# NVlabs/FB-BEV

Hardware: AMD Instinct MI355X
Metric: multi-cam samples/sec (forward view transformation: lift + voxel ranking + bev_pool_v2) (higher is better)
Workload: dtype f32

## Files before the change

fb_bev_amd/csrc/capi.hip:

```cpp
#include <stdio.h>
#include <stdlib.h>
#include <mutex>
#include "rt.h"
#include "pool_kernels.h"
#include "pool_bwd_kernels.h"
#include "rank_kernels.h"
#include "sort_kernels.h"
#include "msda_kernels.h"
#include "geom_kernels.h"
#include "da_kernels.h"
#include "history_kernels.h"
#include "norm_kernels.h"
#include "history_conv_kernels.h"
#include "history_fused_kernels.h"
#include "history_conv_x3_kernels.h"
#include "history_fused_x3_kernels.h"
#include "rows_linear_kernels.h"
#include "rows_linear_f32_kernels.h"
#include "da_fused_kernels.h"
#include "da_bwd_planes_kernels.h"
#include "msda_bwd_kernels.h"
#include "conv3d_kernels.h"
#include "det_kernels.h"
#include "occ_kernels.h"
// ... 102 lines not shown
}

extern "C" int fbbev_tokens_from_nchw_levels(const float* const* in, const int32_t* hw, int n_levels, float* out, int n_images, int C,
                                             const float* bias, int bias_rows, fbbev_stream_t stream_) {
    if (n_levels <= 0 || n_levels > 8 || n_images < 0 || C <= 0 || !in || !hw) return FBBEV_E_BADARG;
    if (bias && bias_rows <= 0) return FBBEV_E_BADARG;
    if (n_images == 0) return 0;
    if (!out) return FBBEV_E_BADARG;
    fbbev_token_levels lv;
    const int tc = (C + 31) / 32;
    long long start = 0, blocks = 0;
    for (int l = 0; l < 8; ++l) { lv.in[l] = nullptr; lv.out_off[l] = 0; lv.hw[l] = 1; lv.blk0[l] = 0; }
    for (int l = 0; l < n_levels; ++l) {
        if (hw[l] <= 0 || !in[l]) return FBBEV_E_BADARG;
        lv.in[l] = in[l]; lv.hw[l] = hw[l]; lv.out_off[l] = start * C; lv.blk0[l] = (int)blocks;
        start += hw[l];
        blocks += (long long)n_images * tc * ((hw[l] + 31) / 32);
        if (blocks >= (1ll << 31)) return FBBEV_E_UNSUPPORTED;
    }
    lv.blk0[n_levels] = (int)blocks;
    lv.n = n_levels;
    FBBEV_LAUNCH(k_nchw_to_nhwc_levels, blocks, 256, 0, (fbbev_rt_stream)stream_, lv, out, C, tc, start * C, bias, bias ? bias_rows : 1);
    FBBEV_CHECK_LAUNCH();
    return 0;
}

extern "C" int fbbev_tokens_from_nchw_pos(const float* in, float* out, int n_images, int C, int HW, long long out_image_stride,
                                          long long out_offset, const float* pos_bias, fbbev_stream_t stream_) {
    if (!pos_bias) return FBBEV_E_BADARG;
    return tokens_from_nchw_impl(in, out, n_images, C, HW, out_image_stride, out_offset, nullptr, 0, pos_bias, stream_);
}

extern "C" int fbbev_point_sampling(const float* xs, const float* ys, const float* zs, const float* rots,
                                    const float* trans, const float* intrins, const float* post_rots,
                                    const float* post_trans, const float* bda, int B, int N, int Y, int X,
                                    int Za, float ogfH, float ogfW, float* ref_cam, uint8_t* mask,
                                    float* qdepth, fbbev_stream_t stream_) {
    if (B <= 0 || N <= 0 || Y <= 0 || X <= 0 || Za <= 0 || !(ogfH > 0.f) || !(ogfW > 0.f)) return FBBEV_E_BADARG;
    if (!xs || !ys || !zs || !rots || !trans || !intrins || !post_rots || !post_trans || !bda || !ref_cam ||
        !mask || !qdepth) return FBBEV_E_BADARG;
    const long long npts = (long long)Y * X * Za;
    int ppt = 8;
    while (ppt > 1 && (npts + 256 * ppt - 1) / (256 * ppt) * B * N < 1024) ppt >>= 1;
    const long long chunks = (npts + 256 * ppt - 1) / (256 * ppt);
    if (chunks * B * N >= (1ll << 31) || ((uintptr_t)ref_cam & 7) != 0) return FBBEV_E_UNSUPPORTED;
    FBBEV_LAUNCH(k_point_sampling, chunks * B * N, 256, 0, (fbbev_rt_stream)stream_, xs, ys, zs, rots, trans,
                 intrins, post_rots, post_trans, bda, B, N, Y, X, Za, ogfH, ogfW, (int)chunks, ref_cam, mask,
                 qdepth, ppt);
    FBBEV_CHECK_LAUNCH();
    return 0;
}

static inline int key_bits(long long total_voxels) {
    int bits = 1;
    while ((1ll << bits) < total_voxels) ++bits;
    return bits;
}

static const int kSortTile[7] = {2048, 4096, 8192, 12288, 16384, 4096, 8192};
static int sort_variant_for(long long items) {
    for (int v = 0; v < 5; ++v)
        if ((items + kSortTile[v] - 1) / kSortTile[v] <= 256) return v;
    return 6;
}
static const int kIvTile[3] = {1024, 4096, 8192};
static int iv_variant_for(long long items) {
    for (int v = 0; v < 3; ++v)
        if ((items + kIvTile[v] - 1) / kIvTile[v] <= 256) return v;
    return 2;
}

static fbbev_fastdiv make_fastdiv(unsigned int d) {
    fbbev_fastdiv f;
    f.d = d; f.m = 0; f.sh = 0;
    if (d <= 1) { f.d = 1; return f; }
    unsigned int l = 0;
    while ((1ull << l) < d) ++l;
    f.m = (unsigned int)((((1ull << l) - d) << 32) / d + 1);
    f.sh = l - 1;
    return f;
}

struct rank_ws_layout {
    size_t keys_a, keys_t, vals_t, matrix, ctot, chunk_info, total;
    int v0, wgs0;
    int v1, wgs1;
    int vi, wgsi;
};

static rank_ws_layout rank_layout(long long n) {
    rank_ws_layout L;
    L.v0 = sort_variant_for(n);
    L.v1 = sort_variant_for((n + 1) / 2);
    L.vi = iv_variant_for((n + 1) / 2);
    if (const char* env = fbbev_env_str("FBBEV_RANK_SHAPE")) {
        int a = -1, b = -1, c = -1;
        if (sscanf(env, "%d,%d,%d", &a, &b, &c) == 3 && a >= 0 && a < 7 && b >= 0 && b < 7 && c >= 0 && c < 3) {
            L.v0 = a; L.v1 = b; L.vi = c;
        }
    }
    L.wgs0 = (int)((n + kSortTile[L.v0] - 1) / kSortTile[L.v0]);
    L.wgs1 = (int)((n + kSortTile[L.v1] - 1) / kSortTile[L.v1]);
    L.wgsi = (int)((n + kIvTile[L.vi] - 1) / kIvTile[L.vi]);
    size_t off = 0;
    L.keys_a = off; off = align_up(off + (size_t)n * 4, 256);
    L.keys_t = off; off = align_up(off + (size_t)n * 4, 256);
    L.vals_t = off; off = align_up(off + (size_t)n * 4, 256);
    const int rows = L.wgs0 > L.wgs1 ? L.wgs0 : L.wgs1;
    const size_t seg_rows = (size_t)(n / FBBEV_SEG_TILE) + 256 + 1;
    size_t mbytes = (size_t)rows * FBBEV_SORT_MAX_NB * 4;
    if (seg_rows * FBBEV_SEG_NB * 4 > mbytes) mbytes = seg_rows * FBBEV_SEG_NB * 4;
    L.matrix = off; off = align_up(off + mbytes, 256);
    L.ctot = off; off = align_up(off + seg_rows * 4, 256);
    L.chunk_info = off; off = align_up(off + (size_t)L.wgsi * 8, 256);
    L.total = off;
    return L;
}

#define FBBEV_SORT_DISPATCH(KERNEL, v, by_waves, grid, stream, ...)                                             \
    do {                                                                                                        \
        switch (v) {                                                                                            \
            case 0: FBBEV_LAUNCH((KERNEL<(by_waves) ? 4 : 256, 8>), grid, 256, 0, stream, __VA_ARGS__); break;   \
            case 1: FBBEV_LAUNCH((KERNEL<(by_waves) ? 16 : 1024, 4>), grid, 1024, 0, stream, __VA_ARGS__); break; \
            case 2: FBBEV_LAUNCH((KERNEL<(by_waves) ? 16 : 1024, 8>), grid, 1024, 0, stream, __VA_ARGS__); break; \
            case 3: FBBEV_LAUNCH((KERNEL<(by_waves) ? 16 : 1024, 12>), grid, 1024, 0, stream, __VA_ARGS__); break; \
            case 5: FBBEV_LAUNCH((KERNEL<(by_waves) ? 8 : 512, 8>), grid, 512, 0, stream, __VA_ARGS__); break;     \
            case 6: FBBEV_LAUNCH((KERNEL<(by_waves) ? 8 : 512, 16>), grid, 512, 0, stream, __VA_ARGS__); break;    \
            default: FBBEV_LAUNCH((KERNEL<(by_waves) ? 16 : 1024, 16>), grid, 1024, 0, stream, __VA_ARGS__); break; \
        }                                                                                                       \
    } while (0)

extern "C" size_t fbbev_rank_workspace_bytes(int64_t n_points) {
    if (n_points <= 0) return 256;
    return rank_layout(n_points).total;
}

static int rank_seg_mode() { FBBEV_KNOB_ONCE(int, m, fbbev_env_int("FBBEV_RANK_SEG", -1)); return m; }

static int rank_build_impl(const float* coor, const fbbev_cam_ptrs* cams, const float* frustum, int B, int N, int D,
                           int H, int W,
                           const float* lower3, const float* interval3, const float* grid_size3,
                           int32_t* ranks_bev, int32_t* ranks_depth, int32_t* ranks_feat,
                           int32_t* interval_starts, int32_t* interval_lengths, int32_t* interval_rank,
                           int32_t* counts, void* workspace, size_t workspace_bytes, fbbev_rt_stream stream,
                           const float* point_depth = nullptr, float depth_thr = 0.f, const int* skip = nullptr) {
    if (B <= 0 || N <= 0 || D <= 0 || H <= 0 || W <= 0) return FBBEV_E_BADARG;
    if (point_depth && cams) return FBBEV_E_UNSUPPORTED;
    if ((!coor && !cams) || !lower3 || !interval3 || !grid_size3 || !ranks_bev || !ranks_depth || !ranks_feat ||
        !interval_starts || !interval_lengths || !counts || !workspace) return FBBEV_E_BADARG;
    const long long n = (long long)B * N * D * H * W;
    if (n >= (1ll << 30)) return FBBEV_E_UNSUPPORTED;
    const rank_ws_layout L = rank_layout(n);
    if (workspace_bytes < L.total) return FBBEV_E_WORKSPACE;
    unsigned char* ws = static_cast<unsigned char*>(workspace);
    unsigned int* keys_a = reinterpret_cast<unsigned int*>(ws + L.keys_a);
    unsigned int* keys_t = reinterpret_cast<unsigned int*>(ws + L.keys_t);
    unsigned int* vals_t = reinterpret_cast<unsigned int*>(ws + L.vals_t);
    int* matrix = reinterpret_cast<int*>(ws + L.matrix);
    int2* chunk_info = reinterpret_cast<int2*>(ws + L.chunk_info);

    fbbev_grid_params gp;
    gp.lx = lower3[0]; gp.ly = lower3[1]; gp.lz = lower3[2];
    gp.ix = interval3[0]; gp.iy = interval3[1]; gp.iz = interval3[2];
    gp.gx = grid_size3[0]; gp.gy = grid_size3[1]; gp.gz = grid_size3[2];
    volatile float zy = gp.gz * gp.gy;
    volatile float zyx = zy * gp.gx;
    volatile float yx = gp.gy * gp.gx;
    gp.f_zyx = zyx; gp.f_yx = yx;
    const long long total_voxels = (long long)B * (long long)gp.gz * (long long)gp.gy * (long long)gp.gx;
    if (total_voxels <= 0 || total_voxels >= (1ll << 30)) return FBBEV_E_UNSUPPORTED;
    const int bits = key_bits(total_voxels + 128);
    struct { int passes, rb; } plan;
    plan.passes = (bits + FBBEV_SORT_MAX_RB - 1) / FBBEV_SORT_MAX_RB;
    plan.rb = (bits + plan.passes - 1) / plan.passes;
    if (plan.rb < 4) plan.rb = 4;
    const int rb = plan.rb;
    const int seg_mode = rank_seg_mode();
    const long long vps = total_voxels / B;
    const long long npb = n / B;
    const int lbits = key_bits(vps);
    const bool seg_legal = B <= 256 && total_voxels <= (1ll << 24) && lbits <= 2 * FBBEV_SEG_RB;
    const long long seg_cps = (npb + FBBEV_SEG_TILE - 1) / FBBEV_SEG_TILE;
    const bool seg = seg_legal && seg_mode != 0 &&
                     (seg_mode == 2 || ((lbits + FBBEV_SEG_RB - 1) / FBBEV_SEG_RB < plan.passes && seg_cps <= 64 && B * seg_cps >= 96));
    if (seg) {
        fbbev_seg sg;
        sg.npb = (int)npb; sg.cps = (int)((npb + FBBEV_SEG_TILE - 1) / FBBEV_SEG_TILE); sg.vps = (unsigned int)vps; sg.nseg = B;
        const int passes = (lbits + FBBEV_SEG_RB - 1) / FBBEV_SEG_RB;
        const int srb = (lbits + passes - 1) / passes < 4 ? 4 : (lbits + passes - 1) / passes;
        const int wgs = B * sg.cps;
        int* ctot = reinterpret_cast<int*>(ws + L.ctot);
        fbbev_geom_src gs;
        if (cams) { gs.cam = *cams; gs.frustum = frustum; gs.gp = gp; }
        else { gs.cam = fbbev_cam_ptrs(); gs.frustum = nullptr; gs.gp = gp; }
        if (cams) FBBEV_LAUNCH((k_keys_hist_seg<true>), wgs, FBBEV_SEG_NT, 0, stream, gs, (const float*)nullptr, gp, (const float*)nullptr, 0.f,
                               sg, srb, skip, keys_a, matrix, ctot);
        else FBBEV_LAUNCH((k_keys_hist_seg<false>), wgs, FBBEV_SEG_NT, 0, stream, gs, coor, gp, point_depth, depth_thr, sg, srb, skip, keys_a,
                          matrix, ctot);
        FBBEV_CHECK_LAUNCH();
        const unsigned int* kin = keys_a;
        const unsigned int* vin = nullptr;
        static const int pairs = fbbev_env_int("FBBEV_RANK_PAIRS", 1);
        for (int p = 0; p < passes; ++p) {
            const bool to_out = p == passes - 1;
            const int pm = pairs ? ((p > 0 ? 1 : 0) | (to_out ? 0 : 2)) : 0;
            unsigned int* ko = to_out ? reinterpret_cast<unsigned int*>(ranks_bev) : keys_t;
            unsigned int* vo = to_out ? reinterpret_cast<unsigned int*>(ranks_depth) : vals_t;
            if (p > 0) {
                FBBEV_LAUNCH(k_sort_hist_seg, wgs, FBBEV_SEG_NT, 0, stream, kin, (const int*)ctot, sg, p * srb, srb, skip, matrix,
                             (pm & 1) ? 2 : 1);
                FBBEV_CHECK_LAUNCH();
            }
            static const int swz = fbbev_env_int("FBBEV_RANK_XCD_SWIZZLE", 1);
            const int sw = (swz && B >= 8) ? 1 : 0;
            FBBEV_LAUNCH(k_sort_scatter_seg, sw ? (wgs + 7) / 8 * 8 : wgs, FBBEV_SEG_NT, 0, stream, kin, vin, (const int*)matrix,
                         (const int*)ctot, sg, p, srb, skip, ko, vo, counts, sw, pm);
            FBBEV_CHECK_LAUNCH();
            kin = ko; vin = vo;
        }
    } else {
    if (cams) {
            fbbev_geom_src gs;
            gs.cam = *cams; gs.frustum = frustum; gs.gp = gp;
            FBBEV_SORT_DISPATCH(k_keys_hist_geom, L.v0, false, L.wgs0, stream, gs, n, rb, skip, keys_a, matrix);
        } else {
            FBBEV_SORT_DISPATCH(k_keys_hist_coor, L.v0, false, L.wgs0, stream, coor, n, n / B, gp, point_depth, depth_thr, rb, keys_a, matrix);
        }
        FBBEV_CHECK_LAUNCH();
        const unsigned int* kin = keys_a;
        const unsigned int* vin = nullptr;
        for (int p = 0; p < plan.passes; ++p) {
            const bool to_out = ((plan.passes - 1 - p) % 2) == 0;
            unsigned int* ko = to_out ? reinterpret_cast<unsigned int*>(ranks_bev) : keys_t;
            unsigned int* vo = to_out ? reinterpret_cast<unsigned int*>(ranks_depth) : vals_t;
            const int v = p == 0 ? L.v0 : L.v1, wgs = p == 0 ? L.wgs0 : L.wgs1;
            if (p > 0) {
                FBBEV_SORT_DISPATCH(k_sort_hist, v, false, wgs, stream, kin, (const int*)counts, p * rb, rb, skip, matrix);
                FBBEV_CHECK_LAUNCH();
            }
            static const int swz = fbbev_env_int("FBBEV_RANK_XCD_SWIZZLE", 1);
            const bool sw = swz == 2 && p == 0;
            FBBEV_SORT_DISPATCH(k_sort_scatter, v, true, sw ? (wgs + 7) / 8 * 8 : wgs, stream, kin, vin, n, (const int*)matrix, p, rb, skip,
                                ko, vo, counts, sw ? wgs : 0);
            FBBEV_CHECK_LAUNCH();
            kin = ko; vin = vo;
        }
}
    const unsigned int* keys = reinterpret_cast<const unsigned int*>(ranks_bev);
    const unsigned int* vals = reinterpret_cast<const unsigned int*>(ranks_depth);
    const fbbev_fastdiv div_dhw = make_fastdiv((unsigned int)((long long)D * H * W)), div_hw = make_fastdiv((unsigned int)(H * W));
    switch (L.vi) {
        case 0:
            FBBEV_LAUNCH((k_interval_count<4, 4>), L.wgsi, 256, 0, stream, keys, (const int*)counts, skip, chunk_info);
            FBBEV_LAUNCH((k_interval_write<4, 4>), L.wgsi, 256, (size_t)2 * 4 * 256 * 4, stream, keys, vals, div_dhw, div_hw, (const int2*)chunk_info, skip,
                         ranks_feat, interval_starts, interval_lengths, interval_rank, counts);
            break;
        case 1:
            FBBEV_LAUNCH((k_interval_count<16, 4>), L.wgsi, 1024, 0, stream, keys, (const int*)counts, skip, chunk_info);
            FBBEV_LAUNCH((k_interval_write<16, 4>), L.wgsi, 1024, (size_t)2 * 4 * 1024 * 4, stream, keys, vals, div_dhw, div_hw, (const int2*)chunk_info, skip,
                         ranks_feat, interval_starts, interval_lengths, interval_rank, counts);
            break;
        default:
            FBBEV_LAUNCH((k_interval_count<16, 8>), L.wgsi, 1024, 0, stream, keys, (const int*)counts, skip, chunk_info);
            FBBEV_LAUNCH((k_interval_write<16, 8>), L.wgsi, 1024, (size_t)2 * 8 * 1024 * 4, stream, keys, vals, div_dhw, div_hw, (const int2*)chunk_info, skip,
                         ranks_feat, interval_starts, interval_lengths, interval_rank, counts);
            break;
    }
    FBBEV_CHECK_LAUNCH();
    return 0;
}

extern "C" int fbbev_rank_build(const float* coor, int B, int N, int D, int H, int W,
                                const float* lower3, const float* interval3,
                                const float* grid_size3, int32_t* ranks_bev, int32_t* ranks_depth,
                                int32_t* ranks_feat, int32_t* interval_starts,
                                int32_t* interval_lengths, int32_t* interval_rank, int32_t* counts,
                                void* workspace, size_t workspace_bytes, fbbev_stream_t stream_) {
    if (!coor) return FBBEV_E_BADARG;
    return rank_build_impl(coor, nullptr, nullptr, B, N, D, H, W, lower3, interval3, grid_size3, ranks_bev, ranks_depth,
                           ranks_feat, interval_starts, interval_lengths, interval_rank, counts, workspace,
                           workspace_bytes, (fbbev_rt_stream)stream_);
}

extern "C" int fbbev_rank_build_depth(const float* coor, const float* depth, float depth_threshold, int B, int N, int D,
                                      int H, int W, const float* lower3, const float* interval3,
                                      const float* grid_size3, int32_t* ranks_bev, int32_t* ranks_depth,
                                      int32_t* ranks_feat, int32_t* interval_starts, int32_t* interval_lengths,
                                      int32_t* interval_rank, int32_t* counts, void* workspace, size_t workspace_bytes,
                                      fbbev_stream_t stream_) {
    if (!coor || !depth) return FBBEV_E_BADARG;
    return rank_build_impl(coor, nullptr, nullptr, B, N, D, H, W, lower3, interval3, grid_size3, ranks_bev, ranks_depth,
                           ranks_feat, interval_starts, interval_lengths, interval_rank, counts, workspace,
                           workspace_bytes, (fbbev_rt_stream)stream_, depth, depth_threshold);
}

static int lift_rank_build_impl(const float* frustum, const float* xs, const float* ys, const float* ds,
                                const float* rots, const float* trans, const float* intrins, const float* post_rots,
                                const float* post_trans, const float* bda, int B, int N, int D, int H, int W,
                                const float* lower3, const float* interval3, const float* grid_size3,
// ... 3383 lines not shown
```

fb_bev_amd/csrc/rank_kernels.h:

```cpp
#pragma once
#include "rt.h"


struct fbbev_grid_params {
    float lx, ly, lz;
    float ix, iy, iz;
    float gx, gy, gz;
    float f_yx, f_zyx;
};

__device__ __forceinline__ unsigned int fbbev_rank_key(float cx, float cy, float cz, const fbbev_grid_params& gp,
                                                       float bf, unsigned int sentinel) {
    const float fx = __fdiv_rn(fbbev_sub(cx, gp.lx), gp.ix);
    const float fy = __fdiv_rn(fbbev_sub(cy, gp.ly), gp.iy);
    const float fz = __fdiv_rn(fbbev_sub(cz, gp.lz), gp.iz);
    const bool finite = (fx == fx) && (fy == fy) && (fz == fz) && fabsf(fx) < 2.0e9f &&
                        fabsf(fy) < 2.0e9f && fabsf(fz) < 2.0e9f;
    const int vx = finite ? (int)fx : -1;
    const int vy = finite ? (int)fy : -1;
    const int vz = finite ? (int)fz : -1;
    const bool kept = finite && vx >= 0 && vy >= 0 && vz >= 0 && (float)vx < gp.gx &&
                      (float)vy < gp.gy && (float)vz < gp.gz;
    float r = fbbev_mul(bf, gp.f_zyx);
    r = fbbev_add(r, fbbev_mul((float)vz, gp.f_yx));
// ... 115 lines not shown
                 int* __restrict__ interval_starts, int* __restrict__ interval_lengths, int* __restrict__ interval_rank,
                 int* __restrict__ counts) {
    if (skip != nullptr && *skip != 0) return;
    constexpr int NT = WAVES * 64;
    constexpr int TILE = NT * ITEMS;
    __shared__ int ldsw[WAVES];
    const int tid = threadIdx.x;
    const int wg = blockIdx.x;
    const int P = counts[0];
    const long long wg0 = (long long)wg * TILE;
    if (wg0 >= P) {
        if (wg == 0 && tid == 0) counts[1] = 0;
        return;
    }
    int h = 0, l1 = 0;
    for (int r = tid; r < wg; r += NT) {
        const int2 ci = chunk_info[r];
        h += ci.x;
        l1 = ci.y > l1 ? ci.y : l1;
    }
    int before_heads, before_last1;
    (void)fbbev_block_excl_scan_w<WAVES, false>(h, ldsw, &before_heads);
    (void)fbbev_block_excl_scan_w<WAVES, true>(l1, ldsw, &before_last1);
    const long long base = wg0 + (long long)tid * ITEMS;
    bool head[ITEMS];
    unsigned int key[ITEMS];
    int local = 0, last1 = 0;
    unsigned int prevk = (base > 0 && base <= P) ? keys[base - 1] : 0u;
    unsigned int pid[ITEMS];
    fbbev_ld_run<ITEMS>(keys, base, P, 0u, key);
    fbbev_ld_run<ITEMS>(vals, base, P, 0u, pid);
    int rf[ITEMS];
#pragma unroll
    for (int j = 0; j < ITEMS; ++j) {
        const long long i = base + j;
        head[j] = false;
        rf[j] = 0;
        if (i < P) {
            const unsigned int k = key[j];
            head[j] = (i == 0 || prevk != k);
            prevk = k;
            if (head[j]) { ++local; last1 = (int)i + 1; }
            const unsigned int cam = fbbev_div(pid[j], div_dhw), hw = pid[j] - fbbev_div(pid[j], div_hw) * div_hw.d;
            rf[j] = (int)(cam * div_hw.d + hw);
        }
    }
    if (base + ITEMS <= P && ((reinterpret_cast<uintptr_t>(ranks_feat + base) & 15u) == 0)) {
#pragma unroll
        for (int q = 0; q < ITEMS / 4; ++q) {
            fbbev_v4i t;
            t[0] = rf[4 * q]; t[1] = rf[4 * q + 1]; t[2] = rf[4 * q + 2]; t[3] = rf[4 * q + 3];
            *reinterpret_cast<fbbev_v4i*>(ranks_feat + base + 4 * q) = t;
        }
    } else {
#pragma unroll
        for (int j = 0; j < ITEMS; ++j)
            if (base + j < P) ranks_feat[base + j] = rf[j];
    }
    int tot, wg_last1;
    const int off = fbbev_block_excl_scan_w<WAVES, false>(local, ldsw, &tot);
    (void)fbbev_block_excl_scan_w<WAVES, true>(last1, ldsw, &wg_last1);
    int* hpos = reinterpret_cast<int*>(fbbev_dyn_lds_f32());
    int* hkey = hpos + TILE;
    {
        int o = off;
#pragma unroll
        for (int j = 0; j < ITEMS; ++j)
            if (head[j]) { hpos[o] = (int)(base + j); hkey[o] = (int)key[j]; ++o; }
    }
    __syncthreads();
    for (int o = tid; o < tot; o += NT) {
        const int pos = hpos[o], j0 = before_heads + o;
        interval_starts[j0] = pos;
        if (interval_rank) interval_rank[j0] = hkey[o];
        if (j0 > 0) interval_lengths[j0 - 1] = pos - (o > 0 ? hpos[o - 1] : before_last1 - 1);
    }
    if (tid == 0 && wg0 + TILE >= P) {
        const int I = before_heads + tot;
        const int lasthead1 = wg_last1 ? wg_last1 : before_last1;
        interval_lengths[I - 1] = P - (lasthead1 - 1);
        counts[1] = I;
    }
}
```

fb_bev_amd/csrc/sort_kernels.h:

```cpp
#pragma once
#include "rt.h"
#include "geom_kernels.h"
#include "rank_kernels.h"

#define FBBEV_SORT_MAX_RB 8
#define FBBEV_SORT_MAX_NB (1 << FBBEV_SORT_MAX_RB)
#define FBBEV_SORT_MAX_PASSES 4
#define FBBEV_DROP_KEY 0xffffffffu

__device__ __forceinline__ bool fbbev_skip(const int* skip) { return skip != nullptr && *skip != 0; }

struct fbbev_geom_src {
    fbbev_cam_ptrs cam;
    const float* frustum;
    fbbev_grid_params gp;
};

__device__ __forceinline__ unsigned int fbbev_geom_key(const fbbev_geom_src& g, const float* m, int cam, int i) {
    float u, v, dep;
    if (g.frustum) {
        u = g.frustum[3 * i]; v = g.frustum[3 * i + 1]; dep = g.frustum[3 * i + 2];
    } else {
        const int w = i % g.cam.W, h = (i / g.cam.W) % g.cam.H, d = i / (g.cam.W * g.cam.H);
        u = g.cam.xs[w]; v = g.cam.ys[h]; dep = g.cam.ds[d];
// ... 167 lines not shown
#pragma unroll
    for (int r = 0; r < ROUNDS; ++r) {
        const long long idx = chunk + r * 64 + lane;
        const bool valid = idx < n;
        k[r] = valid ? keys_in[idx] : FBBEV_DROP_KEY;
        v[r] = valid ? (vals_in ? vals_in[idx] : (unsigned int)idx) : 0u;
    }
#pragma unroll
    for (int r = 0; r < ROUNDS; ++r) {
        const bool valid = k[r] != FBBEV_DROP_KEY;
        lr[r] = -1;
        const unsigned int d = (k[r] >> shift) & dmask;
        unsigned long long mm = __ballot(valid ? 1 : 0);
#pragma unroll
        for (int bit = 0; bit < FBBEV_SORT_MAX_RB; ++bit) {
            if (bit < rb) {
                const unsigned long long b = __ballot((int)((d >> bit) & 1u));
                mm &= ((d >> bit) & 1u) ? b : ~b;
            }
        }
        const int leader = valid ? (__ffsll((long long)mm) - 1) : lane;
        int prev = 0;
        if (valid && lane == leader) {
            prev = cnt[wave][d];
            cnt[wave][d] = prev + __popcll(mm);
        }
        prev = __shfl(prev, leader, 64);
        if (valid) lr[r] = prev + __popcll(mm & lt);
    }
    __syncthreads();
    for (int d = tid; d < nb; d += NT) {
        int run = pos0[d];
#pragma unroll
        for (int w = 0; w < WAVES; ++w) { woff[w][d] = run; run += cnt[w][d]; }
    }
    __syncthreads();
#pragma unroll
    for (int r = 0; r < ROUNDS; ++r) {
        if (lr[r] >= 0) {
            const unsigned int d = (k[r] >> shift) & dmask;
            const int pos = woff[wave][d] + lr[r];
            keys_out[pos] = k[r];
            vals_out[pos] = v[r];
        }
    }
}

#define FBBEV_SEG_RB 10
#define FBBEV_SEG_NB (1 << FBBEV_SEG_RB)
#define FBBEV_SEG_WAVES 8
#define FBBEV_SEG_ROUNDS 16
#define FBBEV_SEG_NT (FBBEV_SEG_WAVES * 64)
#define FBBEV_SEG_TILE (FBBEV_SEG_NT * FBBEV_SEG_ROUNDS)

struct fbbev_seg {
    int npb;
    int cps;
    unsigned int vps;
    int nseg;
};

template <int WAVES>
__device__ __forceinline__ void fbbev_seg_prefix2(const int* __restrict__ ctot, int lo, int hi, int* red, int& sum_lo, int& sum_hi) {
    int a = 0, b = 0;
    for (int i = threadIdx.x; i < hi; i += WAVES * 64) {
        const int c = ctot[i];
        b += c;
        if (i < lo) a += c;
    }
#pragma unroll
    for (int o = 32; o > 0; o >>= 1) { a += __shfl_down(a, o, 64); b += __shfl_down(b, o, 64); }
    const int wave = threadIdx.x >> 6;
    if ((threadIdx.x & 63) == 0) { red[2 * wave] = a; red[2 * wave + 1] = b; }
    __syncthreads();
    sum_lo = 0; sum_hi = 0;
#pragma unroll
    for (int w = 0; w < WAVES; ++w) { sum_lo += red[2 * w]; sum_hi += red[2 * w + 1]; }
    __syncthreads();
}

template <bool GEOM>
__global__ void __launch_bounds__(FBBEV_SEG_NT)
k_keys_hist_seg(fbbev_geom_src g, const float* __restrict__ coor, fbbev_grid_params gp, const float* __restrict__ depth,
                float depth_thr, fbbev_seg sg, int rb, const int* __restrict__ skip, unsigned int* __restrict__ keys_out,
                int* __restrict__ matrix, int* __restrict__ ctot) {
    if (fbbev_skip(skip)) return;
    constexpr int NT = FBBEV_SEG_NT, PER = FBBEV_SEG_ROUNDS;
    __shared__ int cnt[FBBEV_SEG_NB];
    __shared__ float m[33];
    __shared__ int tot;
    const int nb = 1 << rb;
    const unsigned int dmask = (unsigned int)nb - 1u;
    for (int d = threadIdx.x; d < nb; d += NT) cnt[d] = 0;
    if (threadIdx.x == 0) tot = 0;
    const int b = blockIdx.x / sg.cps, c = blockIdx.x - b * sg.cps;
    const int base = b * sg.npb + c * FBBEV_SEG_TILE;
    const int lim = (b + 1) * sg.npb;
    const int end = base + FBBEV_SEG_TILE < lim ? base + FBBEV_SEG_TILE : lim;
    const unsigned int kbase = (unsigned int)b * sg.vps;
    int mine = 0;
    if constexpr (GEOM) {
        const int dhw = g.cam.D * g.cam.H * g.cam.W;
        const int cam_lo = base / dhw, cam_hi = (end > base ? end - 1 : base) / dhw;
        constexpr int G = 8;
        for (int cam = cam_lo; cam <= cam_hi; ++cam) {
            __syncthreads();
            if (threadIdx.x == 0) fbbev_cam_setup(g.cam, cam, m);
            __syncthreads();
            const int c0 = cam * dhw;
            const int lo = base > c0 ? base : c0, hi = end < c0 + dhw ? end : c0 + dhw;
            for (int r0 = 0; r0 < PER; r0 += G) {
                unsigned int key[G];
#pragma unroll
                for (int r = 0; r < G; ++r) {
                    const int pid = base + (int)threadIdx.x + (r0 + r) * NT;
                    key[r] = (pid >= lo && pid < hi) ? fbbev_geom_key(g, m, cam, pid - c0) : FBBEV_DROP_KEY;
                }
#pragma unroll
                for (int r = 0; r < G; ++r) {
                    const int pid = base + (int)threadIdx.x + (r0 + r) * NT;
                    if (pid >= lo && pid < hi) {
                        keys_out[pid] = key[r];
                        if (key[r] != FBBEV_DROP_KEY) { atomicAdd(&cnt[(key[r] - kbase) & dmask], 1); ++mine; }
                    }
                }
            }
        }
    } else {
        __syncthreads();
#pragma unroll
        for (int r = 0; r < PER; ++r) {
            const int pid = base + (int)threadIdx.x + r * NT;
            if (pid < end) {
                unsigned int key = fbbev_rank_key(coor[3 * (long long)pid], coor[3 * (long long)pid + 1], coor[3 * (long long)pid + 2], gp,
                                                  (float)b, FBBEV_DROP_KEY);
                if (depth && !(depth[pid] > depth_thr)) key = FBBEV_DROP_KEY;
                keys_out[pid] = key;
                if (key != FBBEV_DROP_KEY) { atomicAdd(&cnt[(key - kbase) & dmask], 1); ++mine; }
            }
        }
    }
#pragma unroll
    for (int o = 32; o > 0; o >>= 1) mine += __shfl_down(mine, o, 64);
    if ((threadIdx.x & 63) == 0 && mine) atomicAdd(&tot, mine);
    __syncthreads();
    for (int d = threadIdx.x; d < nb; d += NT) matrix[(long long)blockIdx.x * nb + d] = cnt[d];
    if (threadIdx.x == 0) ctot[blockIdx.x] = tot;
}

__global__ void __launch_bounds__(FBBEV_SEG_NT)
k_sort_hist_seg(const unsigned int* __restrict__ keys, const int* __restrict__ ctot, fbbev_seg sg, int shift, int rb,
                const int* __restrict__ skip, int* __restrict__ matrix, int key_stride) {
    if (fbbev_skip(skip)) return;
    constexpr int NT = FBBEV_SEG_NT, PER = FBBEV_SEG_ROUNDS;
    __shared__ int cnt[FBBEV_SEG_NB];
    __shared__ int red[2 * FBBEV_SEG_WAVES];
    const int nb = 1 << rb;
    const unsigned int dmask = (unsigned int)nb - 1u;
    const int b = blockIdx.x / sg.cps, c = blockIdx.x - b * sg.cps;
    for (int d = threadIdx.x; d < nb; d += NT) cnt[d] = 0;
    int s0, s1;
    fbbev_seg_prefix2<FBBEV_SEG_WAVES>(ctot, b * sg.cps, (b + 1) * sg.cps, red, s0, s1);
    const long long base = (long long)s0 + (long long)c * FBBEV_SEG_TILE;
    const unsigned int kbase = (unsigned int)b * sg.vps;
    if (base < s1) {
        unsigned int key[PER];
#pragma unroll
        for (int r = 0; r < PER; ++r) {
            const long long idx = base + threadIdx.x + r * NT;
            key[r] = (idx < s1) ? keys[idx * key_stride] : FBBEV_DROP_KEY;
        }
#pragma unroll
        for (int r = 0; r < PER; ++r)
            if (key[r] != FBBEV_DROP_KEY) atomicAdd(&cnt[((key[r] - kbase) >> shift) & dmask], 1);
    }
    __syncthreads();
    for (int d = threadIdx.x; d < nb; d += NT) matrix[(long long)blockIdx.x * nb + d] = cnt[d];
}

__global__ void __launch_bounds__(FBBEV_SEG_NT)
k_sort_scatter_seg(const unsigned int* __restrict__ keys_in, const unsigned int* __restrict__ vals_in, const int* __restrict__ matrix,
                   const int* __restrict__ ctot, fbbev_seg sg, int pass, int rb, const int* __restrict__ skip,
                   unsigned int* __restrict__ keys_out, unsigned int* __restrict__ vals_out, int* __restrict__ counts, int xcd_swizzle, int pair_mode) {
    if (fbbev_skip(skip)) return;
    constexpr int WAVES = FBBEV_SEG_WAVES, ROUNDS = FBBEV_SEG_ROUNDS, NT = FBBEV_SEG_NT, NBM = FBBEV_SEG_NB;
    int chunk_id = (int)blockIdx.x;
    if (xcd_swizzle) {
        const int total = sg.nseg * sg.cps, per_xcd = (total + 7) >> 3;
        chunk_id = (int)(blockIdx.x & 7) * per_xcd + (int)(blockIdx.x >> 3);
        if (chunk_id >= total) return;
    }
    __shared__ __attribute__((aligned(16))) int cnt[WAVES][NBM];
    __shared__ int pos0[NBM];
    __shared__ int red[2 * WAVES];
    __shared__ int ldsw[WAVES];
    const int tid = threadIdx.x, wave = tid >> 6, lane = tid & 63;
    const int nb = 1 << rb, shift = pass * rb;
    const unsigned int dmask = (unsigned int)nb - 1u;
    const int b = chunk_id / sg.cps, c = chunk_id - b * sg.cps;
    const unsigned int kbase = (unsigned int)b * sg.vps;
    int s0, s1;
    fbbev_seg_prefix2<WAVES>(ctot, b * sg.cps, (b + 1) * sg.cps, red, s0, s1);
    if (pass == 0 && chunk_id == 0) {
        int p0, pall;
        fbbev_seg_prefix2<WAVES>(ctot, 0, sg.nseg * sg.cps, red, p0, pall);
        if (tid == 0) counts[0] = pall;
    }
    const long long in0 = pass == 0 ? (long long)b * sg.npb : (long long)s0;
    const long long in1 = pass == 0 ? (long long)(b + 1) * sg.npb : (long long)s1;
    const long long chunk0 = in0 + (long long)c * FBBEV_SEG_TILE;
    if (chunk0 >= in1) return;
    const long long chunk = chunk0 + (long long)wave * (64 * ROUNDS);
    unsigned int k[ROUNDS], v[ROUNDS];
    int lr[ROUNDS];
    const unsigned long long lt = (lane == 0) ? 0ull : (~0ull >> (64 - lane));
#pragma unroll
    for (int r = 0; r < ROUNDS; ++r) {
        const long long idx = chunk + r * 64 + lane;
        const bool valid = idx < in1;
        if (pair_mode & 1) {
            uint2 kv = make_uint2(FBBEV_DROP_KEY, 0u);
            if (valid) kv = reinterpret_cast<const uint2*>(keys_in)[idx];
            k[r] = kv.x; v[r] = kv.y;
        } else {
            k[r] = valid ? keys_in[idx] : FBBEV_DROP_KEY;
            v[r] = valid ? (vals_in ? vals_in[idx] : (unsigned int)idx) : 0u;
        }
    }
    const int row0 = b * sg.cps;
    {
        const int nq = nb >> 2;
        const int quad = tid % nq, rg = tid / nq;
        fbbev_v4i pre = {0, 0, 0, 0}, all = {0, 0, 0, 0};
        if (rg < 2) {
            constexpr int U = 8;
            const int* col = matrix + (long long)row0 * nb + 4 * quad;
            for (int r = rg; r < sg.cps; r += 2 * U) {
                fbbev_v4i t[U];
#pragma unroll
                for (int u = 0; u < U; ++u) {
                    const int rr = r + 2 * u < sg.cps ? r + 2 * u : sg.cps - 1;
                    __builtin_memcpy(&t[u], col + (long long)rr * nb, 16);
                }
#pragma unroll
                for (int u = 0; u < U; ++u) {
                    if (r + 2 * u < sg.cps) all += t[u];
                    if (r + 2 * u < c) pre += t[u];
                }
            }
            __builtin_memcpy(&cnt[1 + rg][4 * quad], &pre, 16);
            __builtin_memcpy(&cnt[3 + rg][4 * quad], &all, 16);
        }
    }
    __syncthreads();
    {
        const int d0 = 2 * tid, d1 = 2 * tid + 1;
        const int a0 = d0 < nb ? cnt[3][d0] + cnt[4][d0] : 0, a1 = d1 < nb ? cnt[3][d1] + cnt[4][d1] : 0;
        const int p0 = d0 < nb ? cnt[1][d0] + cnt[2][d0] : 0, p1 = d1 < nb ? cnt[1][d1] + cnt[2][d1] : 0;
        int total;
        const int ex = fbbev_block_excl_scan_w<WAVES, false>(a0 + a1, ldsw, &total);
        if (d0 < nb) pos0[d0] = p0 + s0 + ex;
        if (d1 < nb) pos0[d1] = p1 + s0 + ex + a0;
    }
    __syncthreads();
    for (int i = tid; i < WAVES * NBM; i += NT) (&cnt[0][0])[i] = 0;
    __syncthreads();
#pragma unroll
    for (int r = 0; r < ROUNDS; ++r) {
        const bool valid = k[r] != FBBEV_DROP_KEY;
        lr[r] = -1;
        const unsigned int d = ((k[r] - kbase) >> shift) & dmask;
        unsigned long long mm = __ballot(valid ? 1 : 0);
#pragma unroll
        for (int bit = 0; bit < FBBEV_SEG_RB; ++bit) {
            if (bit < rb) {
                const unsigned long long bb = __ballot((int)((d >> bit) & 1u));
                mm &= ((d >> bit) & 1u) ? bb : ~bb;
            }
        }
        const int leader = valid ? (__ffsll((long long)mm) - 1) : lane;
        int prev = 0;
        if (valid && lane == leader) {
            prev = cnt[wave][d];
            cnt[wave][d] = prev + __popcll(mm);
        }
        prev = __shfl(prev, leader, 64);
        if (valid) lr[r] = prev + __popcll(mm & lt);
    }
    __syncthreads();
    for (int d = tid; d < nb; d += NT) {
        int run = pos0[d];
#pragma unroll
        for (int w = 0; w < WAVES; ++w) { const int t = cnt[w][d]; cnt[w][d] = run; run += t; }
    }
    __syncthreads();
#pragma unroll
    for (int r = 0; r < ROUNDS; ++r) {
        if (lr[r] >= 0) {
            const unsigned int d = ((k[r] - kbase) >> shift) & dmask;
            const int pos = cnt[wave][d] + lr[r];
            if (pair_mode & 2) reinterpret_cast<uint2*>(keys_out)[pos] = make_uint2(k[r], v[r]);
            else { keys_out[pos] = k[r]; vals_out[pos] = v[r]; }
        }
    }
}

__global__ void __launch_bounds__(256)
k_cam_key(fbbev_cam_ptrs g, int B, unsigned int* __restrict__ key, int* __restrict__ state) {
    __shared__ int differ;
    if (threadIdx.x == 0) differ = 0;
    __syncthreads();
    const int cams = B * g.N;
    const float* src[6] = {g.rots, g.trans, g.intrins, g.post_rots, g.post_trans, g.bda};
    const int len[6] = {cams * 9, cams * 3, cams * 9, cams * 9, cams * 3, B * 9};
    int off = 0, bad = 0;
    for (int s = 0; s < 6; ++s) {
        for (int i = threadIdx.x; i < len[s]; i += 256) {
            unsigned int bits;
            const float f = src[s][i];
            __builtin_memcpy(&bits, &f, 4);
            bad |= (bits != key[off + i]) ? 1 : 0;
        }
        off += len[s];
    }
    if (bad) differ = 1;
    __syncthreads();
    if (!differ) { if (threadIdx.x == 0) state[0] = 1; return; }
    off = 0;
    for (int s = 0; s < 6; ++s) {
        for (int i = threadIdx.x; i < len[s]; i += 256) {
            unsigned int bits;
            const float f = src[s][i];
            __builtin_memcpy(&bits, &f, 4);
            key[off + i] = bits;
        }
        off += len[s];
    }
    if (threadIdx.x == 0) { state[0] = 0; state[1] += 1; }
}
```

Before: 23150.

## Replace second radix pass with bucket-local finish sort and fused interval extraction

When the segmented rank sort needs two passes, the first pass now buckets by the high key bits, and a new bucket-finish kernel sorts each bucket by its low bits. The finish kernel uses one wave per short bucket and a whole workgroup per long bucket, and it writes ranks_bev/depth/feat directly while counting per-bucket interval heads. A new interval kernel then uses those per-bucket head counts to emit interval starts, lengths and ranks without a global scan pass. This is meant to remove the second global scatter pass and the separate gather/interval stages, at the cost of extra workspace and more complex kernels that depend on how bucket sizes are distributed.

New measurement: 23800, median of 6. 2.8% higher.

```diff
diff --git a/fb_bev_amd/csrc/capi.hip b/fb_bev_amd/csrc/capi.hip
--- a/fb_bev_amd/csrc/capi.hip
+++ b/fb_bev_amd/csrc/capi.hip
@@ -208,7 +208,7 @@
 }
 
 struct rank_ws_layout {
-    size_t keys_a, keys_t, vals_t, matrix, ctot, chunk_info, total;
+    size_t keys_a, keys_t, vals_t, matrix, ctot, chunk_info, boff, hb, total;
     int v0, wgs0;
     int v1, wgs1;
     int vi, wgsi;
@@ -239,6 +239,9 @@
     L.matrix = off; off = align_up(off + mbytes, 256);
     L.ctot = off; off = align_up(off + seg_rows * 4, 256);
     L.chunk_info = off; off = align_up(off + (size_t)L.wgsi * 8, 256);
+    const size_t fin_buckets = (size_t)(n < 256 ? n : 256) * FBBEV_SEG_NB;
+    L.boff = off; off = align_up(off + (fin_buckets + 1) * 4, 256);
+    L.hb = off; off = align_up(off + fin_buckets * 4, 256);
     L.total = off;
     return L;
 }
@@ -262,6 +265,11 @@
 }
 
 static int rank_seg_mode() { FBBEV_KNOB_ONCE(int, m, fbbev_env_int("FBBEV_RANK_SEG", -1)); return m; }
+static int rank_finish_mode() { FBBEV_KNOB_ONCE(int, m, fbbev_env_int("FBBEV_RANK_FINISH", -1)); return m; }
+static bool rank_finish_auto(int lbits, long long npb, int B) {
+    (void)npb; (void)B;
+    return lbits >= 2 * FBBEV_SEG_RB;
+}
 
 static int rank_build_impl(const float* coor, const fbbev_cam_ptrs* cams, const float* frustum, int B, int N, int D,
                            int H, int W,
@@ -319,11 +327,41 @@
         fbbev_geom_src gs;
         if (cams) { gs.cam = *cams; gs.frustum = frustum; gs.gp = gp; }
         else { gs.cam = fbbev_cam_ptrs(); gs.frustum = nullptr; gs.gp = gp; }
+        const int fin_mode = rank_finish_mode();
+        const bool finish = passes == 2 && fin_mode != 0 && (fin_mode == 1 || rank_finish_auto(lbits, npb, B));
+        const int high_bits = FBBEV_SEG_RB, low_bits = lbits - FBBEV_SEG_RB;
+        const int rb0 = finish ? high_bits : srb, dshift0 = finish ? low_bits : 0;
         if (cams) FBBEV_LAUNCH((k_keys_hist_seg<true>), wgs, FBBEV_SEG_NT, 0, stream, gs, (const float*)nullptr, gp, (const float*)nullptr, 0.f,
-                               sg, srb, skip, keys_a, matrix, ctot);
-        else FBBEV_LAUNCH((k_keys_hist_seg<false>), wgs, FBBEV_SEG_NT, 0, stream, gs, coor, gp, point_depth, depth_thr, sg, srb, skip, keys_a,
-                          matrix, ctot);
+                               sg, rb0, dshift0, skip, keys_a, matrix, ctot);
+        else FBBEV_LAUNCH((k_keys_hist_seg<false>), wgs, FBBEV_SEG_NT, 0, stream, gs, coor, gp, point_depth, depth_thr, sg, rb0, dshift0, skip,
+                          keys_a, matrix, ctot);
         FBBEV_CHECK_LAUNCH();
+        if (finish) {
+            int* boff = reinterpret_cast<int*>(ws + L.boff);
+            int* hb = reinterpret_cast<int*>(ws + L.hb);
+            const int nbk = (int)((vps + (1ll << low_bits) - 1) >> low_bits);
+            const int buckets = B * nbk;
+            static const int swz = fbbev_env_int("FBBEV_RANK_XCD_SWIZZLE", 1);
+            const int sw = (swz && B >= 8) ? 1 : 0;
+            FBBEV_LAUNCH(k_sort_scatter_seg, sw ? (wgs + 7) / 8 * 8 : wgs, FBBEV_SEG_NT, 0, stream, (const unsigned int*)keys_a,
+                         (const unsigned int*)nullptr, (const int*)matrix, (const int*)ctot, sg, 0, high_bits, skip, keys_t, vals_t, counts, sw, 2,
+                         low_bits, boff, nbk);
+            FBBEV_CHECK_LAUNCH();
+            const fbbev_fastdiv div_dhw = make_fastdiv((unsigned int)((long long)D * H * W)), div_hw = make_fastdiv((unsigned int)(H * W));
+            int short_wgs = (buckets + FBBEV_FIN_WAVES - 1) / FBBEV_FIN_WAVES;
+            if (short_wgs > 2048) short_wgs = 2048;
+            const int long_wgs = buckets < 512 ? buckets : 512;
+            FBBEV_LAUNCH(k_bucket_finish, long_wgs + short_wgs, FBBEV_FIN_WAVES * 64, 0, stream, reinterpret_cast<const uint2*>(keys_t),
+                         (const int*)boff, buckets, nbk, sg.vps, low_bits, long_wgs, div_dhw, div_hw, skip,
+                         reinterpret_cast<unsigned int*>(ranks_bev), reinterpret_cast<unsigned int*>(ranks_depth), ranks_feat, hb);
+            FBBEV_CHECK_LAUNCH();
+            const int per_wg = (buckets + 255) / 256;
+            FBBEV_LAUNCH((k_bucket_intervals<16, 4>), (buckets + per_wg - 1) / per_wg, 1024, (size_t)2 * 4 * 1024 * 4, stream,
+                         reinterpret_cast<const unsigned int*>(ranks_bev), (const int*)boff, (const int*)hb, buckets, per_wg, skip,
+                         interval_starts, interval_lengths, interval_rank, counts);
+            FBBEV_CHECK_LAUNCH();
+            return 0;
+        }
         const unsigned int* kin = keys_a;
         const unsigned int* vin = nullptr;
         static const int pairs = fbbev_env_int("FBBEV_RANK_PAIRS", 1);
@@ -340,7 +378,7 @@
             static const int swz = fbbev_env_int("FBBEV_RANK_XCD_SWIZZLE", 1);
             const int sw = (swz && B >= 8) ? 1 : 0;
             FBBEV_LAUNCH(k_sort_scatter_seg, sw ? (wgs + 7) / 8 * 8 : wgs, FBBEV_SEG_NT, 0, stream, kin, vin, (const int*)matrix,
-                         (const int*)ctot, sg, p, srb, skip, ko, vo, counts, sw, pm);
+                         (const int*)ctot, sg, p, srb, skip, ko, vo, counts, sw, pm, -1, (int*)nullptr, 0);
             FBBEV_CHECK_LAUNCH();
             kin = ko; vin = vo;
         }
diff --git a/fb_bev_amd/csrc/rank_kernels.h b/fb_bev_amd/csrc/rank_kernels.h
--- a/fb_bev_amd/csrc/rank_kernels.h
+++ b/fb_bev_amd/csrc/rank_kernels.h
@@ -221,3 +221,80 @@
         counts[1] = I;
     }
 }
+
+template <int WAVES, int ITEMS>
+__global__ void __launch_bounds__(WAVES * 64)
+k_bucket_intervals(const unsigned int* __restrict__ keys, const int* __restrict__ boff, const int* __restrict__ hb, int buckets,
+                   int per_wg, const int* __restrict__ skip, int* __restrict__ interval_starts, int* __restrict__ interval_lengths,
+                   int* __restrict__ interval_rank, int* __restrict__ counts) {
+    if (skip != nullptr && *skip != 0) return;
+    constexpr int NT = WAVES * 64;
+    constexpr int TILE = NT * ITEMS;
+    __shared__ int ldsw[WAVES];
+    const int tid = threadIdx.x;
+    const int g0 = (int)blockIdx.x * per_wg;
+    if (g0 >= buckets) return;
+    const int g1 = g0 + per_wg < buckets ? g0 + per_wg : buckets;
+    const int r0 = boff[g0], r1 = boff[g1];
+    int h = 0;
+    {
+        constexpr int U = 4;
+        const int nq = g0 >> 2;
+        const fbbev_v4i* hb4 = reinterpret_cast<const fbbev_v4i*>(hb);
+        for (int q0 = tid; q0 < nq; q0 += NT * U) {
+            fbbev_v4i t[U];
+#pragma unroll
+            for (int u = 0; u < U; ++u) {
+                const int qi = q0 + u * NT;
+                t[u] = hb4[qi < nq ? qi : nq - 1];
+            }
+#pragma unroll
+            for (int u = 0; u < U; ++u)
+                if (q0 + u * NT < nq) h += t[u][0] + t[u][1] + t[u][2] + t[u][3];
+        }
+        if (tid < (g0 & 3)) h += hb[4 * nq + tid];
+    }
+    int hbase;
+    (void)fbbev_block_excl_scan_w<WAVES, false>(h, ldsw, &hbase);
+    int* hpos = reinterpret_cast<int*>(fbbev_dyn_lds_f32());
+    int* hkey = hpos + TILE;
+    int lastpos = r0;
+    for (int t0 = r0; t0 < r1; t0 += TILE) {
+        const long long base = (long long)t0 + (long long)tid * ITEMS;
+        bool head[ITEMS];
+        unsigned int key[ITEMS];
+        int local = 0;
+        unsigned int prevk = (base > r0 && base <= r1) ? keys[base - 1] : 0u;
+        fbbev_ld_run<ITEMS>(keys, base, r1, 0u, key);
+#pragma unroll
+        for (int j = 0; j < ITEMS; ++j) {
+            const long long i = base + j;
+            head[j] = false;
+            if (i < r1) {
+                head[j] = (i == r0 || prevk != key[j]);
+                prevk = key[j];
+                if (head[j]) ++local;
+            }
+        }
+        int tot;
+        int o = fbbev_block_excl_scan_w<WAVES, false>(local, ldsw, &tot);
+#pragma unroll
+        for (int j = 0; j < ITEMS; ++j)
+            if (head[j]) { hpos[o] = (int)(base + j); hkey[o] = (int)key[j]; ++o; }
+        __syncthreads();
+        for (int q = tid; q < tot; q += NT) {
+            const int pos = hpos[q], j0 = hbase + q;
+            interval_starts[j0] = pos;
+            if (interval_rank) interval_rank[j0] = hkey[q];
+            if (q > 0) interval_lengths[j0 - 1] = pos - hpos[q - 1];
+            else if (t0 > r0) interval_lengths[j0 - 1] = pos - lastpos;
+        }
+        if (tot > 0) lastpos = hpos[tot - 1];
+        hbase += tot;
+        __syncthreads();
+    }
+    if (tid == 0) {
+        if (r1 > r0) interval_lengths[hbase - 1] = r1 - lastpos;
+        if (g1 == buckets) counts[1] = hbase;
+    }
+}
diff --git a/fb_bev_amd/csrc/sort_kernels.h b/fb_bev_amd/csrc/sort_kernels.h
--- a/fb_bev_amd/csrc/sort_kernels.h
+++ b/fb_bev_amd/csrc/sort_kernels.h
@@ -273,7 +273,7 @@
 template <bool GEOM>
 __global__ void __launch_bounds__(FBBEV_SEG_NT)
 k_keys_hist_seg(fbbev_geom_src g, const float* __restrict__ coor, fbbev_grid_params gp, const float* __restrict__ depth,
-                float depth_thr, fbbev_seg sg, int rb, const int* __restrict__ skip, unsigned int* __restrict__ keys_out,
+                float depth_thr, fbbev_seg sg, int rb, int dshift, const int* __restrict__ skip, unsigned int* __restrict__ keys_out,
                 int* __restrict__ matrix, int* __restrict__ ctot) {
     if (fbbev_skip(skip)) return;
     constexpr int NT = FBBEV_SEG_NT, PER = FBBEV_SEG_ROUNDS;
@@ -312,7 +312,7 @@
                     const int pid = base + (int)threadIdx.x + (r0 + r) * NT;
                     if (pid >= lo && pid < hi) {
                         keys_out[pid] = key[r];
-                        if (key[r] != FBBEV_DROP_KEY) { atomicAdd(&cnt[(key[r] - kbase) & dmask], 1); ++mine; }
+                        if (key[r] != FBBEV_DROP_KEY) { atomicAdd(&cnt[((key[r] - kbase) >> dshift) & dmask], 1); ++mine; }
                     }
                 }
             }
@@ -327,7 +327,7 @@
                                                   (float)b, FBBEV_DROP_KEY);
                 if (depth && !(depth[pid] > depth_thr)) key = FBBEV_DROP_KEY;
                 keys_out[pid] = key;
-                if (key != FBBEV_DROP_KEY) { atomicAdd(&cnt[(key - kbase) & dmask], 1); ++mine; }
+                if (key != FBBEV_DROP_KEY) { atomicAdd(&cnt[((key - kbase) >> dshift) & dmask], 1); ++mine; }
             }
         }
     }
@@ -372,7 +372,8 @@
 __global__ void __launch_bounds__(FBBEV_SEG_NT)
 k_sort_scatter_seg(const unsigned int* __restrict__ keys_in, const unsigned int* __restrict__ vals_in, const int* __restrict__ matrix,
                    const int* __restrict__ ctot, fbbev_seg sg, int pass, int rb, const int* __restrict__ skip,
-                   unsigned int* __restrict__ keys_out, unsigned int* __restrict__ vals_out, int* __restrict__ counts, int xcd_swizzle, int pair_mode) {
+                   unsigned int* __restrict__ keys_out, unsigned int* __restrict__ vals_out, int* __restrict__ counts, int xcd_swizzle, int pair_mode,
+                   int dshift, int* __restrict__ boff, int nbk) {
     if (fbbev_skip(skip)) return;
     constexpr int WAVES = FBBEV_SEG_WAVES, ROUNDS = FBBEV_SEG_ROUNDS, NT = FBBEV_SEG_NT, NBM = FBBEV_SEG_NB;
     int chunk_id = (int)blockIdx.x;
@@ -386,7 +387,7 @@
     __shared__ int red[2 * WAVES];
     __shared__ int ldsw[WAVES];
     const int tid = threadIdx.x, wave = tid >> 6, lane = tid & 63;
-    const int nb = 1 << rb, shift = pass * rb;
+    const int nb = 1 << rb, shift = dshift >= 0 ? dshift : pass * rb;
     const unsigned int dmask = (unsigned int)nb - 1u;
     const int b = chunk_id / sg.cps, c = chunk_id - b * sg.cps;
     const unsigned int kbase = (unsigned int)b * sg.vps;
@@ -395,7 +396,7 @@
     if (pass == 0 && chunk_id == 0) {
         int p0, pall;
         fbbev_seg_prefix2<WAVES>(ctot, 0, sg.nseg * sg.cps, red, p0, pall);
-        if (tid == 0) counts[0] = pall;
+        if (tid == 0) { counts[0] = pall; if (boff) boff[sg.nseg * nbk] = pall; }
     }
     const long long in0 = pass == 0 ? (long long)b * sg.npb : (long long)s0;
     const long long in1 = pass == 0 ? (long long)(b + 1) * sg.npb : (long long)s1;
@@ -452,6 +453,10 @@
         const int ex = fbbev_block_excl_scan_w<WAVES, false>(a0 + a1, ldsw, &total);
         if (d0 < nb) pos0[d0] = p0 + s0 + ex;
         if (d1 < nb) pos0[d1] = p1 + s0 + ex + a0;
+        if (boff && c == 0) {
+            if (d0 < nbk) boff[b * nbk + d0] = s0 + ex;
+            if (d1 < nbk) boff[b * nbk + d1] = s0 + ex + a0;
+        }
     }
     __syncthreads();
     for (int i = tid; i < WAVES * NBM; i += NT) (&cnt[0][0])[i] = 0;
@@ -492,6 +497,166 @@
             const int pos = cnt[wave][d] + lr[r];
             if (pair_mode & 2) reinterpret_cast<uint2*>(keys_out)[pos] = make_uint2(k[r], v[r]);
             else { keys_out[pos] = k[r]; vals_out[pos] = v[r]; }
+        }
+    }
+}
+
+#define FBBEV_FIN_WAVES 4
+#define FBBEV_FIN_STAGE 8
+#define FBBEV_FIN_SLOT(d) ((d) + ((d) >> 4))
+#define FBBEV_FIN_WORDS (FBBEV_SEG_NB + (FBBEV_SEG_NB >> 4))
+
+__global__ void __launch_bounds__(FBBEV_FIN_WAVES * 64)
+k_bucket_finish(const uint2* __restrict__ pairs, const int* __restrict__ boff, int buckets, int nbk, unsigned int vps, int low_bits,
+                int long_wgs, fbbev_fastdiv div_dhw, fbbev_fastdiv div_hw, const int* __restrict__ skip,
+                unsigned int* __restrict__ ranks_bev, unsigned int* __restrict__ ranks_depth, int* __restrict__ ranks_feat,
+                int* __restrict__ hb) {
+    if (fbbev_skip(skip)) return;
+    constexpr int WAVES = FBBEV_FIN_WAVES, ST = FBBEV_FIN_STAGE, NT = FBBEV_FIN_WAVES * 64;
+    __shared__ int cntw[WAVES][FBBEV_FIN_WORDS];
+    __shared__ int lds4[4];
+    const int tid = threadIdx.x, wave = tid >> 6, lane = tid & 63;
+    const int nlow = 1 << low_bits;
+    const unsigned int lmask = (unsigned int)nlow - 1u;
+    const unsigned long long lt = (lane == 0) ? 0ull : (~0ull >> (64 - lane));
+    uint2 kv[ST];
+    auto load = [&](int g0, int end) {
+#pragma unroll
+        for (int r = 0; r < ST; ++r) {
+            const int idx = g0 + r * 64 + lane;
+            kv[r] = make_uint2(FBBEV_DROP_KEY, 0u);
+            if (idx < end) kv[r] = pairs[idx];
+        }
+    };
+    auto count = [&](unsigned int kbase) {
+#pragma unroll
+        for (int r = 0; r < ST; ++r)
+            if (kv[r].x != FBBEV_DROP_KEY) atomicAdd(&cntw[wave][FBBEV_FIN_SLOT((int)((kv[r].x - kbase) & lmask))], 1);
+    };
+    auto rank = [&](int g0, int end, int start, unsigned int kbase) {
+#pragma unroll
+        for (int r = 0; r < ST; ++r) {
+            if (g0 + r * 64 < end) {
+                const bool valid = kv[r].x != FBBEV_DROP_KEY;
+                const unsigned int d = (kv[r].x - kbase) & lmask;
+                unsigned long long mm = __ballot(valid ? 1 : 0);
+#pragma unroll
+                for (int bit = 0; bit < FBBEV_SEG_RB; ++bit) {
+                    const unsigned long long bb = __ballot((int)((d >> bit) & 1u));
+                    mm &= ((d >> bit) & 1u) ? bb : ~bb;
+                }
+                const int leader = valid ? (__ffsll((long long)mm) - 1) : lane;
+                int prev = 0;
+                if (valid && lane == leader) {
+                    prev = cntw[wave][FBBEV_FIN_SLOT((int)d)];
+                    cntw[wave][FBBEV_FIN_SLOT((int)d)] = prev + __popcll(mm);
+                }
+                prev = __shfl(prev, leader, 64);
+                if (valid) {
+                    const int pos = start + prev + __popcll(mm & lt);
+                    const unsigned int pid = kv[r].y;
+                    const unsigned int cam = fbbev_div(pid, div_dhw), hw = pid - fbbev_div(pid, div_hw) * div_hw.d;
+                    ranks_bev[pos] = kv[r].x;
+                    ranks_depth[pos] = pid;
+                    ranks_feat[pos] = (int)(cam * div_hw.d + hw);
+                }
+                fbbev_sched_fence();
+            }
+        }
+    };
+
+    if ((int)blockIdx.x >= long_wgs) {
+        const int short_wgs = (int)gridDim.x - long_wgs, sw = (int)blockIdx.x - long_wgs;
+        const int per = nlow >= 64 ? nlow >> 6 : 1;
+        for (int g = sw * WAVES + wave; g < buckets; g += short_wgs * WAVES) {
+            const int start = boff[g], end = boff[g + 1];
+            if (end <= start) {
+                if (lane == 0) hb[g] = 0;
+                continue;
+            }
+            if (end - start > 64 * ST) continue;
+            const unsigned int kbase = (unsigned int)(g / nbk) * vps;
+            load(start, end);
+            for (int d = lane; d < nlow; d += 64) cntw[wave][FBBEV_FIN_SLOT(d)] = 0;
+            fbbev_wave_sync();
+            count(kbase);
+            fbbev_wave_sync();
+            int sum = 0, nz = 0;
+            if (lane * per < nlow) {
+                for (int j = 0; j < per; ++j) {
+                    const int c = cntw[wave][FBBEV_FIN_SLOT(lane * per + j)];
+                    sum += c;
+                    nz += c != 0 ? 1 : 0;
+                }
+            }
+            int run = fbbev_wave_incl_scan(sum, lane) - sum;
+            if (lane * per < nlow) {
+                for (int j = 0; j < per; ++j) {
+                    const int c = cntw[wave][FBBEV_FIN_SLOT(lane * per + j)];
+                    cntw[wave][FBBEV_FIN_SLOT(lane * per + j)] = run;
+                    run += c;
+                }
+            }
+#pragma unroll
+            for (int o = 32; o > 0; o >>= 1) nz += __shfl_down(nz, o, 64);
+            if (lane == 0) hb[g] = nz;
+            fbbev_wave_sync();
+            rank(start, end, start, kbase);
+            fbbev_wave_sync();
+        }
+        return;
+    }
+    const int L = (int)blockIdx.x;
+    const int per = nlow >= NT ? nlow / NT : 1;
+    for (int base = L; base < buckets; base += 64 * long_wgs) {
+        const int mine = base + lane * long_wgs;
+        const bool is_long = mine < buckets && boff[mine + 1] - boff[mine] > 64 * ST;
+        unsigned long long todo = __ballot(is_long ? 1 : 0);
+        while (todo) {
+            const int l = __ffsll((long long)todo) - 1;
+            todo &= todo - 1;
+            const int g = base + l * long_wgs;
+            const int start = boff[g], end = boff[g + 1];
+            const unsigned int kbase = (unsigned int)(g / nbk) * vps;
+            const int q = ((end - start + 64 * WAVES - 1) / (64 * WAVES)) * 64;
+            const int w0 = start + wave * q < end ? start + wave * q : end, w1 = w0 + q < end ? w0 + q : end;
+            for (int d = lane; d < nlow; d += 64) cntw[wave][FBBEV_FIN_SLOT(d)] = 0;
+            fbbev_wave_sync();
+            for (int g0 = w0; g0 < w1; g0 += 64 * ST) {
+                load(g0, w1);
+                count(kbase);
+            }
+            __syncthreads();
+            int sum = 0, nz = 0;
+            if (tid * per < nlow) {
+                for (int j = 0; j < per; ++j) {
+                    int c = 0;
+#pragma unroll
+                    for (int w = 0; w < WAVES; ++w) c += cntw[w][FBBEV_FIN_SLOT(tid * per + j)];
+                    sum += c;
+                    nz += c != 0 ? 1 : 0;
+                }
+            }
+            int total, heads;
+            int run = fbbev_block_excl_scan(sum, lds4, &total);
+            (void)fbbev_block_excl_scan(nz, lds4, &heads);
+            if (tid * per < nlow) {
+                for (int j = 0; j < per; ++j) {
+#pragma unroll
+                    for (int w = 0; w < WAVES; ++w) {
+                        const int c = cntw[w][FBBEV_FIN_SLOT(tid * per + j)];
+                        cntw[w][FBBEV_FIN_SLOT(tid * per + j)] = run;
+                        run += c;
+                    }
+                }
+            }
+            if (tid == 0) hb[g] = heads;
+            __syncthreads();
+            for (int g0 = w0; g0 < w1; g0 += 64 * ST) {
+                load(g0, w1);
+                rank(g0, w1, start, kbase);
+            }
+            __syncthreads();
         }
     }
 }
```
